# santi-pdp/segan_pytorch

Hardware: AMD Instinct MI355X
Metric: 16384-sample waveform chunks/sec (GAN step) (higher is better)
Workload: dtype f32

## Files before the change

include/segan_hip.h:

```cpp
#ifndef SEGAN_HIP_H
#define SEGAN_HIP_H

#include <stddef.h>
#include <stdint.h>

#ifdef __cplusplus
extern "C" {
#endif

#define SEGAN_ABI_VERSION 17

#define SEGAN_PAD_REFLECT 0
#define SEGAN_PAD_ZERO 1

#define SEGAN_ACT_NONE 0
#define SEGAN_ACT_TANH 1

typedef struct segan_src {
  const float* p0;
  const float* p1;
  int32_t C0;
  int32_t C1;
  const float* scale;
  const float* shift;
// ... 40 lines not shown

int segan_deconv1d_fwd(const segan_src* x, const void* wt, const float* w, const float* bias,
                       float* y, int B, int M, int N, int Ls, int K, int S, int pad, int act,
                       int precision, void* scratch, size_t scratch_bytes, void* stream);

int segan_deconv1d_dgrad(const float* dy, const void* wf, float* dx0, float* dx1, int B, int M,
                         int M0, int N, int Ls, int K, int S, int pad, int precision, void* scratch,
                         size_t scratch_bytes, void* stream);


int segan_bn_nsplit(int B, int C, int L);
int segan_bn_stats(const float* x, const float* gamma, const float* beta, float eps,
                   float momentum, float* running_mean, float* running_var, float* mean,
                   float* rstd, float* scale, float* shift, float* ws, int B, int C, int L,
                   void* stream);
int segan_bn_partial(const float* x, float* ws, int B, int C, int L, void* stream);
int segan_bn_final(const float* ws, int nsplit_total, const float* gamma, const float* beta,
                   float eps, float momentum, float* running_mean, float* running_var, float* mean,
                   float* rstd, float* scale, float* shift, int C, void* stream);

int segan_affine_tanh(const float* x, const float* scale, const float* shift, float* y, int B,
                      int C, int L, void* stream);
int segan_scale_mask(const float* x, const float* scale, const float* mask, float* y, int B, int C,
                     int L, void* stream);

int segan_affine_prelu(const float* x, const float* scale, const float* shift, const float* slope,
                       float* y, int B, int C, int L, void* stream);

int segan_sum_skip(const float* x0, const float* slope0, const float* x1, const float* alpha,
                   float* out, int B, int C, int L, void* stream);
// ... 169 lines not shown
```

segan_pytorch_amd/_lib.py:

```python
import ctypes
import os
from ctypes import POINTER, Structure, c_char_p, c_double, c_float, c_int, c_int32, c_int64, c_size_t, c_void_p

_HERE = os.path.dirname(os.path.abspath(__file__))
LIB_PATH = os.environ.get('SEGAN_HIP_LIB') or os.path.join(_HERE, 'libsegan_hip.so')

PAD_REFLECT = 0
PAD_ZERO = 1
ACT_NONE = 0
ACT_TANH = 1
ABI_VERSION = 17


class SeganSrc(Structure):
    _fields_ = [('p0', c_void_p), ('p1', c_void_p), ('C0', c_int32), ('C1', c_int32),
                ('scale', c_void_p), ('shift', c_void_p), ('slope', c_void_p)]


_P = c_void_p
_SRC = POINTER(SeganSrc)

SIGNATURES = {
    'segan_abi_version': (c_int, []),
    'segan_set_reserved_slots': (c_int, [c_int]),
# ... 9 lines not shown
    'segan_debug_last_wgrad': (None, [POINTER(c_int)]),
    'segan_conv1d_fwd': (c_int, [_SRC, _P, _P, _P, c_int, c_int, c_int, c_int, c_int, c_int, c_int,
                                 c_int, c_int, c_int, _P, c_size_t, _P]),
    'segan_conv1d_dgrad': (c_int, [_P, _P, _P, _P, _P, c_int, c_int, c_int, c_int, c_int, c_int, c_int,
                                   c_int, c_int, _P, c_size_t, _P]),
    'segan_wgrad': (c_int, [_SRC, _SRC, _P, c_int, c_int, c_int, c_int, c_int, c_int, c_int, c_int,
                            c_int, c_int, c_int, _P, c_size_t, _P]),
    'segan_wgrad_scratch_bytes': (c_size_t, [c_int, c_int, c_int, c_int, c_int, c_int, c_int]),
    'segan_deconv1d_fwd': (c_int, [_SRC, _P, _P, _P, _P, c_int, c_int, c_int, c_int, c_int, c_int, c_int,
                                   c_int, c_int, _P, c_size_t, _P]),
    'segan_deconv1d_dgrad': (c_int, [_P, _P, _P, _P, c_int, c_int, c_int, c_int, c_int, c_int, c_int,
                                     c_int, c_int, _P, c_size_t, _P]),
    'segan_bn_nsplit': (c_int, [c_int, c_int, c_int]),
    'segan_bn_stats': (c_int, [_P, _P, _P, c_float, c_float, _P, _P, _P, _P, _P, _P, _P, c_int, c_int,
                               c_int, _P]),
    'segan_bn_partial': (c_int, [_P, _P, c_int, c_int, c_int, _P]),
    'segan_bn_final': (c_int, [_P, c_int, _P, _P, c_float, c_float, _P, _P, _P, _P, _P, _P, c_int, _P]),
    'segan_act_bwd_bn_reduce': (c_int, [_P] * 12 + [c_int, c_int, c_int, _P]),
    'segan_act_bwd_bn_apply': (c_int, [_P] * 11 + [c_int, c_int, c_int, c_double, _P]),
    'segan_affine_prelu': (c_int, [_P, _P, _P, _P, _P, c_int, c_int, c_int, _P]),
    'segan_affine_tanh': (c_int, [_P, _P, _P, _P, c_int, c_int, c_int, _P]),
    'segan_scale_mask': (c_int, [_P, _P, _P, _P, c_int, c_int, c_int, _P]),
    'segan_sum_skip': (c_int, [_P, _P, _P, _P, _P, c_int, c_int, c_int, _P]),
    'segan_bce_logits_const': (c_int, [_P, c_float, _P, _P, _P, c_float, c_int, _P]),
    'segan_act_bwd': (c_int, [_P] * 16 + [c_int, c_int, c_int, _P]),
    'segan_tanh_bwd': (c_int, [_P, _P, _P, c_float, _P, _P, _P, c_int, c_int, c_int, _P]),
    'segan_gemm_scratch_bytes': (c_size_t, [c_int, c_int, c_int]),
    'segan_gemm': (c_int, [_P, c_int64, c_int64, _P, c_int64, c_int64, _P, c_int64, c_int, c_int,
                           c_int, c_int, c_int, _P, c_size_t, _P]),
    'segan_bias_prelu_rows': (c_int, [_P, _P, _P, _P, c_int, c_int, _P]),
# ... 105 lines not shown
```

segan_pytorch_amd/csrc/segan_pointwise.hip:

```cpp
#include "segan_common.h"

#define PW_THREADS 256

static int pw_nsplit(int B, int C, int L) {
  int ns = ceil_div(2048, C);
  if (ns > B) ns = B;
  long per = (long)B * L / ns;
  while (ns > 1 && per < 2048) {
    ns = (ns + 1) / 2;
    per = (long)B * L / ns;
  }
  return ns < 1 ? 1 : ns;
}

extern "C" int segan_bn_nsplit(int B, int C, int L) {
  if (B <= 0 || C <= 0 || L <= 0) return 0;
  return pw_nsplit(B, C, L);
}

template <int NV>
__device__ __forceinline__ void block_sum(float (&v)[NV], float* sm) {
  const int lane = threadIdx.x & 63, wave = threadIdx.x >> 6;
#pragma unroll
  for (int k = 0; k < NV; ++k) v[k] = warp_sum(v[k]);
// ... 23 lines not shown
  r.b_end = min(B, r.b_beg + per);
  return r;
}

__device__ __forceinline__ void chan_combine(float& n, float& mean, float& m2, float nb, float mb,
                                             float qb) {
  const float tot = n + nb;
  if (tot <= 0.0f) return;
  const float d = mb - mean;
  const float f = nb / tot;
  mean = fmaf(d, f, mean);
  m2 = m2 + qb + d * d * n * f;
  n = tot;
}

__global__ void bn_partial_kernel(const float* __restrict__ x, float* __restrict__ ws, int B, int C,
                                  int L, int nsplit) {
  __shared__ float sm[3 * (PW_THREADS / 64)];
  const ChanRange cr = chan_range(B, nsplit);
  const int nb = cr.b_end - cr.b_beg;
  const float* base = x + ((size_t)cr.b_beg * C + cr.c) * L;
  const size_t sstride = (size_t)C * L;
  const bool vec = (L & 3) == 0 && ((uintptr_t)x & 15) == 0;
  const int Lv = vec ? L >> 2 : L;
  int tr = PW_THREADS;
  while (tr > Lv && tr > 1) tr >>= 1;
  const int rp = PW_THREADS / tr;
  const int t0 = threadIdx.x % tr, r0 = threadIdx.x / tr;
  float K = 0.0f, s1 = 0.0f, s2 = 0.0f, n = 0.0f;
  if (r0 < nb && t0 < Lv) K = base[(size_t)r0 * sstride + (vec ? 4 * t0 : t0)];
  for (int b = r0; b < nb; b += rp) {
    const float* row = base + b * sstride;
// ... 24 lines not shown
    m2 = fmaxf(s2 - s1 * r, 0.0f);
  }
#pragma unroll
  for (int o = 32; o > 0; o >>= 1) {
    const float nb2 = __shfl_down(n, o, 64), mb2 = __shfl_down(mean, o, 64), qb2 = __shfl_down(m2, o, 64);
    chan_combine(n, mean, m2, nb2, mb2, qb2);
  }
  const int lane = threadIdx.x & 63, wave = threadIdx.x >> 6;
  if (lane == 0) {
    sm[3 * wave] = n; sm[3 * wave + 1] = mean; sm[3 * wave + 2] = m2;
  }
  __syncthreads();
  if (threadIdx.x == 0) {
    for (int w = 1; w < PW_THREADS / 64; ++w) chan_combine(n, mean, m2, sm[3 * w], sm[3 * w + 1], sm[3 * w + 2]);
    float* w = ws + ((size_t)blockIdx.y * C + cr.c) * 3;
    w[0] = n;
    w[1] = mean;
    w[2] = m2;
  }
}

__device__ __forceinline__ void bn_affine(float gamma, float beta, float mean, float rstd,
                                          float& scale, float& shift) {
  scale = gamma * rstd;
  shift = fmaf(-mean, scale, beta);
}

__global__ void bn_final_kernel(const float* __restrict__ ws, const float* gamma, const float* beta,
                                float eps, float momentum, float* running_mean, float* running_var,
                                float* mean_o, float* rstd_o, float* scale_o, float* shift_o, int C,
                                int nsplit) {
  const int c = blockIdx.x * blockDim.x + threadIdx.x;
  if (c >= C) return;
  double n = 0.0, mean = 0.0, m2 = 0.0;
  for (int s = 0; s < nsplit; ++s) {
    const float* w = ws + ((size_t)s * C + c) * 3;
    const double nb = w[0], mb = w[1], qb = w[2];
    if (nb <= 0.0) continue;
    const double tot = n + nb;
    const double d = mb - mean;
    mean += d * nb / tot;
    m2 += qb + d * d * n * nb / tot;
    n = tot;
  }
  const double var = n > 0 ? m2 / n : 0.0;
  const float rstd = (float)(1.0 / sqrt(var + (double)eps));
  const float g = gamma ? gamma[c] : 1.0f;
  const float bt = beta ? beta[c] : 0.0f;
  float sc, sh;
  bn_affine(g, bt, (float)mean, rstd, sc, sh);
  if (mean_o) mean_o[c] = (float)mean;
  if (rstd_o) rstd_o[c] = rstd;
  if (scale_o) scale_o[c] = sc;
  if (shift_o) shift_o[c] = sh;
  if (running_mean) running_mean[c] = (1.0f - momentum) * running_mean[c] + momentum * (float)mean;
  if (running_var) {
    const double unb = n > 1 ? m2 / (n - 1.0) : var;
    running_var[c] = (1.0f - momentum) * running_var[c] + momentum * (float)unb;
  }
}

extern "C" int segan_bn_stats(const float* x, const float* gamma, const float* beta, float eps,
                              float momentum, float* running_mean, float* running_var, float* mean,
                              float* rstd, float* scale, float* shift, float* ws, int B, int C,
                              int L, void* stream) {
  SEGAN_REQUIRE(x && ws, "bn_stats: NULL pointer");
  SEGAN_REQUIRE(B > 0 && C > 0 && L > 0, "bn_stats: bad sizes");
  hipStream_t st = (hipStream_t)stream;
  const int ns = pw_nsplit(B, C, L);
  hipLaunchKernelGGL(bn_partial_kernel, dim3(C, ns), dim3(PW_THREADS), 0, st, x, ws, B, C, L, ns);
  hipLaunchKernelGGL(bn_final_kernel, dim3(ceil_div(C, 64)), dim3(64), 0, st, ws, gamma, beta, eps,
                     momentum, running_mean, running_var, mean, rstd, scale, shift, C, ns);
  return segan_check_launch("bn_stats");
}

extern "C" int segan_bn_partial(const float* x, float* ws, int B, int C, int L, void* stream) {
  SEGAN_REQUIRE(x && ws, "bn_partial: NULL pointer");
  SEGAN_REQUIRE(B > 0 && C > 0 && L > 0, "bn_partial: bad sizes");
  const int ns = pw_nsplit(B, C, L);
  hipLaunchKernelGGL(bn_partial_kernel, dim3(C, ns), dim3(PW_THREADS), 0, (hipStream_t)stream, x, ws,
                     B, C, L, ns);
  return segan_check_launch("bn_partial");
}

extern "C" int segan_bn_final(const float* ws, int nsplit_total, const float* gamma,
                              const float* beta, float eps, float momentum, float* running_mean,
                              float* running_var, float* mean, float* rstd, float* scale,
                              float* shift, int C, void* stream) {
  SEGAN_REQUIRE(ws && nsplit_total > 0 && C > 0, "bn_final: bad arguments");
  hipLaunchKernelGGL(bn_final_kernel, dim3(ceil_div(C, 64)), dim3(64), 0, (hipStream_t)stream, ws,
                     gamma, beta, eps, momentum, running_mean, running_var, mean, rstd, scale, shift,
                     C, nsplit_total);
  return segan_check_launch("bn_final");
}

__global__ void affine_prelu_kernel(const float* __restrict__ x, const float* scale,
                                    const float* shift, const float* slope, float* __restrict__ y,
                                    size_t total, int C, int L) {
  for (size_t i = blockIdx.x * (size_t)blockDim.x + threadIdx.x; i < total;
       i += (size_t)gridDim.x * blockDim.x) {
    const int c = (int)((i / L) % C);
    float v = x[i];
    v = fmaf(v, scale ? scale[c] : 1.0f, shift ? shift[c] : 0.0f);
    if (slope) v = v > 0.f ? v : v * slope[c];
    y[i] = v;
  }
// ... 77 lines not shown

struct ActBwdArgs {
  const float* a;
  const float* dh;
  const float* dskip;
  const float* slope;
  const float* alpha;
  const float* mean;
  const float* rstd;
  const float* gamma;
  const float* beta;
  float* da;
  float* ws;
  int B, C, L, nsplit;
  float inv_count;
};

template <int PHASE>
__global__ void act_bwd_kernel(const ActBwdArgs p) {
  __shared__ float sm[16];
  const ChanRange cr = chan_range(p.B, p.nsplit);
  const int c = cr.c;
  const int nb = cr.b_end - cr.b_beg;
  const float sl = p.slope ? p.slope[c] : 1.0f;
  const float al = p.alpha ? p.alpha[c] : 0.0f;
  float mu = 0.f, rs = 1.f, ga = 1.f, be = 0.f, dbeta_m = 0.f, dgamma_m = 0.f, sc = 1.f, sh = 0.f;
  if (PHASE != 0) {
    mu = p.mean[c];
    rs = p.rstd[c];
    ga = p.gamma ? p.gamma[c] : 1.0f;
    be = p.beta ? p.beta[c] : 0.0f;
    bn_affine(ga, be, mu, rs, sc, sh);
  }
  if (PHASE == 2) {
    const float* tot = p.ws + (size_t)p.nsplit * p.C * 4 + (size_t)c * 2;
    dbeta_m = tot[0] * p.inv_count;
    dgamma_m = tot[1] * p.inv_count;
  }
  float r[3] = {0.f, 0.f, 0.f};
  const bool has_skip = p.dskip != nullptr;
  auto elem = [&](float av, float dh, float ds) -> float {
    if (PHASE == 0) {
      float g = dh * (av > 0.f ? 1.0f : sl);
      r[0] += dh * (av > 0.f ? 0.0f : av);
      if (has_skip) {
        g = fmaf(al, ds, g);
        r[1] = fmaf(ds, av, r[1]);
      }
      r[2] += g;
      return g;
    }
    const float xh = (av - mu) * rs;
// ... 29 lines not shown
        const f32x4 ds = has_skip ? *reinterpret_cast<const f32x4*>(p.dskip + i) : z4;
        f32x4 o;
#pragma unroll
        for (int e = 0; e < 4; ++e) o[e] = elem(av[e], dh[e], ds[e]);
        if (PHASE != 1) *reinterpret_cast<f32x4*>(p.da + i) = o;
      }
    } else {
      for (int t = t0; t < Lv; t += tr) {
        const size_t i = ro + t;
        const float o = elem(p.a[i], p.dh ? p.dh[i] : 0.0f, has_skip ? p.dskip[i] : 0.0f);
        if (PHASE != 1) p.da[i] = o;
      }
    }
  }
  block_sum<3>(r, sm);
  if (threadIdx.x == 0) {
    float* w = p.ws + ((size_t)blockIdx.y * p.C + c) * 4;
    w[0] = r[0];
    w[1] = r[1];
    w[2] = r[2];
  }
}

template <int PHASE>
__global__ void act_bwd_final_kernel(const ActBwdArgs p, float* dslope, float* dalpha,
                                     float* dgamma, float* dbeta, float* dbias) {
  const int c = blockIdx.x * blockDim.x + threadIdx.x;
  if (c >= p.C) return;
  float s0 = 0.f, s1 = 0.f, s2 = 0.f;
  for (int s = 0; s < p.nsplit; ++s) {
    const float* w = p.ws + ((size_t)s * p.C + c) * 4;
    s0 += w[0];
    s1 += w[1];
    s2 += w[2];
  }
// ... 13 lines not shown
  }
}

extern "C" int segan_act_bwd(const float* a, const float* dh, const float* dskip,
                             const float* slope, const float* alpha, const float* bn_mean,
                             const float* bn_rstd, const float* bn_gamma, const float* bn_beta,
                             float* da, float* dslope, float* dalpha, float* dgamma, float* dbeta,
                             float* dbias, float* ws, int B, int C, int L, void* stream) {
  SEGAN_REQUIRE(a && da && ws, "act_bwd: NULL pointer");
  SEGAN_REQUIRE(dh || dskip, "act_bwd: no incoming gradient");
  SEGAN_REQUIRE(B > 0 && C > 0 && L > 0, "act_bwd: bad sizes");
  SEGAN_REQUIRE((bn_mean == nullptr) == (bn_rstd == nullptr), "act_bwd: mean/rstd must pair");
  SEGAN_REQUIRE(!(dskip && !alpha), "act_bwd: dskip needs alpha");
  SEGAN_REQUIRE(!(bn_mean && dskip), "act_bwd: BN layers have no skip tap");
  hipStream_t st = (hipStream_t)stream;
  ActBwdArgs p;
  p.a = a; p.dh = dh; p.dskip = dskip; p.slope = slope; p.alpha = alpha;
  p.mean = bn_mean; p.rstd = bn_rstd; p.gamma = bn_gamma; p.beta = bn_beta;
  p.da = da; p.ws = ws; p.B = B; p.C = C; p.L = L;
  p.nsplit = pw_nsplit(B, C, L);
  p.inv_count = 1.0f / ((float)B * (float)L);
  const dim3 grid(C, p.nsplit), fgrid(ceil_div(C, 64));
  if (!bn_mean) {
    hipLaunchKernelGGL(act_bwd_kernel<0>, grid, dim3(PW_THREADS), 0, st, p);
    hipLaunchKernelGGL(act_bwd_final_kernel<0>, fgrid, dim3(64), 0, st, p, dslope, dalpha, dgamma,
                       dbeta, dbias);
  } else {
    hipLaunchKernelGGL(act_bwd_kernel<1>, grid, dim3(PW_THREADS), 0, st, p);
    hipLaunchKernelGGL(act_bwd_final_kernel<1>, fgrid, dim3(64), 0, st, p, dslope, dalpha, dgamma,
                       dbeta, dbias);
    hipLaunchKernelGGL(act_bwd_kernel<2>, grid, dim3(PW_THREADS), 0, st, p);
    hipLaunchKernelGGL(act_bwd_final_kernel<2>, fgrid, dim3(64), 0, st, p, dslope, dalpha, dgamma,
                       dbeta, dbias);
  }
  return segan_check_launch("act_bwd");
}

extern "C" int segan_act_bwd_bn_reduce(const float* a, const float* dh, const float* slope,
                                       const float* bn_mean, const float* bn_rstd,
                                       const float* bn_gamma, const float* bn_beta, float* dslope,
                                       float* dgamma, float* dbeta, float* totals, float* ws, int B,
                                       int C, int L, void* stream) {
  SEGAN_REQUIRE(a && dh && bn_mean && bn_rstd && totals && ws, "act_bwd_bn_reduce: NULL pointer");
  SEGAN_REQUIRE(B > 0 && C > 0 && L > 0, "act_bwd_bn_reduce: bad sizes");
  hipStream_t st = (hipStream_t)stream;
  ActBwdArgs p;
  p.a = a; p.dh = dh; p.dskip = nullptr; p.slope = slope; p.alpha = nullptr;
  p.mean = bn_mean; p.rstd = bn_rstd; p.gamma = bn_gamma; p.beta = bn_beta;
  p.da = nullptr; p.ws = ws; p.B = B; p.C = C; p.L = L;
  p.nsplit = pw_nsplit(B, C, L);
  p.inv_count = 1.0f / ((float)B * (float)L);
  hipLaunchKernelGGL(act_bwd_kernel<1>, dim3(C, p.nsplit), dim3(PW_THREADS), 0, st, p);
  hipLaunchKernelGGL(act_bwd_final_kernel<1>, dim3(ceil_div(C, 64)), dim3(64), 0, st, p, dslope,
                     (float*)nullptr, dgamma, dbeta, (float*)nullptr);
  if (hipMemcpyAsync(totals, ws + (size_t)p.nsplit * C * 4, (size_t)C * 2 * sizeof(float),
                     hipMemcpyDeviceToDevice, st) != hipSuccess) {
    segan_set_error("act_bwd_bn_reduce: copy of the totals failed");
    return SEGAN_ELAUNCH;
  }
  return segan_check_launch("act_bwd_bn_reduce");
}

extern "C" int segan_act_bwd_bn_apply(const float* a, const float* dh, const float* slope,
                                      const float* bn_mean, const float* bn_rstd,
                                      const float* bn_gamma, const float* bn_beta,
                                      const float* totals, float* da, float* dbias, float* ws, int B,
                                      int C, int L, double count_total, void* stream) {
  SEGAN_REQUIRE(a && dh && bn_mean && bn_rstd && totals && da && ws, "act_bwd_bn_apply: NULL pointer");
  SEGAN_REQUIRE(B > 0 && C > 0 && L > 0 && count_total >= (double)B * L, "act_bwd_bn_apply: bad sizes");
  hipStream_t st = (hipStream_t)stream;
  ActBwdArgs p;
  p.a = a; p.dh = dh; p.dskip = nullptr; p.slope = slope; p.alpha = nullptr;
  p.mean = bn_mean; p.rstd = bn_rstd; p.gamma = bn_gamma; p.beta = bn_beta;
  p.da = da; p.ws = ws; p.B = B; p.C = C; p.L = L;
  p.nsplit = pw_nsplit(B, C, L);
  p.inv_count = (float)(1.0 / count_total);
  if (hipMemcpyAsync(ws + (size_t)p.nsplit * C * 4, totals, (size_t)C * 2 * sizeof(float),
                     hipMemcpyDeviceToDevice, st) != hipSuccess) {
    segan_set_error("act_bwd_bn_apply: copy of the totals failed");
    return SEGAN_ELAUNCH;
  }
  hipLaunchKernelGGL(act_bwd_kernel<2>, dim3(C, p.nsplit), dim3(PW_THREADS), 0, st, p);
  hipLaunchKernelGGL(act_bwd_final_kernel<2>, dim3(ceil_div(C, 64)), dim3(64), 0, st, p,
                     (float*)nullptr, (float*)nullptr, (float*)nullptr, (float*)nullptr, dbias);
  return segan_check_launch("act_bwd_bn_apply");
}

__global__ void tanh_bwd_kernel(const float* __restrict__ y, const float* dy, const float* clean,
                                float l1_scale, float* __restrict__ da, float* ws, int B, int C,
                                int L, int nsplit) {
  __shared__ float sm[16];
  const ChanRange cr = chan_range(B, nsplit);
  const int nb = cr.b_end - cr.b_beg;
  const long cnt = (long)(nb > 0 ? nb : 0) * L;
  float r[1] = {0.f};
  for (long e = threadIdx.x; e < cnt; e += PW_THREADS) {
    const int b = cr.b_beg + (int)(e / L);
    const int t = (int)(e % L);
    const size_t i = ((size_t)b * C + cr.c) * L + t;
    const float yv = y[i];
    float g = dy ? dy[i] : 0.0f;
    if (clean) {
      const float d = yv - clean[i];
      g += l1_scale * (d > 0.f ? 1.0f : (d < 0.f ? -1.0f : 0.0f));
    }
    const float d = g * (1.0f - yv * yv);
    da[i] = d;
    r[0] += d;
  }
  block_sum<1>(r, sm);
  if (threadIdx.x == 0) ws[(size_t)blockIdx.y * C + cr.c] = r[0];
}

__global__ void sum_splits_add_kernel(const float* ws, float* out, int C, int nsplit) {
  const int c = blockIdx.x * blockDim.x + threadIdx.x;
  if (c >= C) return;
  float s = 0.f;
  for (int k = 0; k < nsplit; ++k) s += ws[(size_t)k * C + c];
  out[c] += s;
}

extern "C" int segan_tanh_bwd(const float* y, const float* dy, const float* clean, float l1_scale,
                              float* da, float* dbias, float* ws, int B, int C, int L,
                              void* stream) {
  SEGAN_REQUIRE(y && da && ws, "tanh_bwd: NULL pointer");
  SEGAN_REQUIRE(dy || clean, "tanh_bwd: no incoming gradient");
  SEGAN_REQUIRE(B > 0 && C > 0 && L > 0, "tanh_bwd: bad sizes");
  hipStream_t st = (hipStream_t)stream;
  const int ns = pw_nsplit(B, C, L);
  hipLaunchKernelGGL(tanh_bwd_kernel, dim3(C, ns), dim3(PW_THREADS), 0, st, y, dy, clean, l1_scale,
                     da, ws, B, C, L, ns);
  if (dbias)
    hipLaunchKernelGGL(sum_splits_add_kernel, dim3(ceil_div(C, 64)), dim3(64), 0, st, ws, dbias, C,
                       ns);
  return segan_check_launch("tanh_bwd");
}

__global__ void bias_prelu_rows_kernel(const float* __restrict__ x, const float* bias,
                                       const float* slope, float* __restrict__ y, int rows,
                                       int cols) {
  const size_t total = (size_t)rows * cols;
  for (size_t i = blockIdx.x * (size_t)blockDim.x + threadIdx.x; i < total;
       i += (size_t)gridDim.x * blockDim.x) {
    const int c = (int)(i % cols);
    float v = x[i] + (bias ? bias[c] : 0.0f);
    if (slope) v = v > 0.f ? v : v * slope[c];
    y[i] = v;
// ... 30 lines not shown
      s_b += d;
      dx[i] = d;
    }
  }
  sm[0][rg][cl] = s_sl;
  sm[1][rg][cl] = s_b;
  __syncthreads();
  if (rg == 0 && c < cols) {
    const float a = sm[0][0][cl] + sm[0][1][cl] + sm[0][2][cl] + sm[0][3][cl];
    const float b = sm[1][0][cl] + sm[1][1][cl] + sm[1][2][cl] + sm[1][3][cl];
    if (dslope && slope) dslope[c] += a;
    if (dbias) dbias[c] += b;
  }
}

extern "C" int segan_bias_prelu_rows_bwd(const float* x, const float* bias, const float* slope,
                                         const float* dy, float* dx, float* dslope, float* dbias,
                                         int rows, int cols, void* stream) {
  SEGAN_REQUIRE(x && dy && dx && rows > 0 && cols > 0, "bias_prelu_rows_bwd: bad arguments");
  hipLaunchKernelGGL(bias_prelu_rows_bwd_kernel, dim3(ceil_div(cols, 64)), dim3(256), 0,
                     (hipStream_t)stream, x, bias, slope, dy, dx, dslope, dbias, rows, cols);
  return segan_check_launch("bias_prelu_rows_bwd");
}

__global__ void mse_const_kernel(const float* __restrict__ x, float target, float* loss,
                                 float* grad, const float* gout, float gscale, int n) {
  __shared__ float sm[16];
  float r[1] = {0.f};
  const float inv = 1.0f / (float)n;
  if (gout) gscale *= gout[0];
  for (int i = threadIdx.x; i < n; i += PW_THREADS) {
    const float d = x[i] - target;
    r[0] = fmaf(d, d, r[0]);
    if (grad) grad[i] = 2.0f * d * inv * gscale;
  }
  block_sum<1>(r, sm);
// ... 288 lines not shown
```

segan_pytorch_amd/functional.py:

```python
import os

import torch

from . import ops
from .ops import ACT_NONE, ACT_TANH, PAD_REFLECT, PAD_ZERO, Src


def grad_buf(p):
    if p.grad is None:
        p.grad = torch.zeros_like(p, memory_format=torch.contiguous_format)
    elif not p.grad.is_contiguous():
        p.grad = p.grad.contiguous()
    return p.grad


def _gb(p, needed=True):
    if p is None or not needed or not p.requires_grad:
        return None
    return grad_buf(p)


def _bn_batch_stats(bn, training):
    return training or bn.running_mean is None or bn.running_var is None


def _bn_train_stats(c, bn, training=True):
    from . import distributed as sdist
    fn = sdist.bn_stats_sync if sdist.sync_bn_enabled() else ops.bn_stats
    track = training and bn.running_mean is not None and bn.running_var is not None
    momentum = 0.0
    if track:
        if bn.num_batches_tracked is not None:
            bn.num_batches_tracked += 1
        if bn.momentum is not None:
            momentum = bn.momentum
        else:
            momentum = 1.0 / float(bn.num_batches_tracked) if bn.num_batches_tracked is not None else 0.0
    return fn(c, bn.weight, bn.bias, bn.eps, momentum, bn.running_mean if track else None,
              bn.running_var if track else None)


def _bn_eval_affine(bn):
    rstd = torch.rsqrt(bn.running_var + bn.eps)
    gamma = bn.weight.detach() if bn.weight is not None else torch.ones_like(rstd)
    beta = bn.bias.detach() if bn.bias is not None else torch.zeros_like(rstd)
    scale = (gamma * rstd).contiguous()
# ... 816 lines not shown
```

segan_pytorch_amd/ops.py:

```python
import ctypes
import operator

import torch

from . import _lib
from . import layout
from ._lib import ACT_NONE, ACT_TANH, PAD_REFLECT, PAD_ZERO, SeganSrc, check


import os as _os

PREC_FP32, PREC_BF16, PREC_BF16X3 = 0, 1, 3
_PREC_NAMES = {'fp32': PREC_FP32, 'bf16': PREC_BF16, 'bf16x3': PREC_BF16X3}
_precision = _PREC_NAMES[_os.environ.get('SEGAN_PRECISION', 'fp32')]
_EUNSUPPORTED = -3


_deterministic = _os.environ.get('SEGAN_DETERMINISTIC', '0') == '1'


def set_deterministic(on):
    global _deterministic
    _deterministic = bool(on)

# ... 434 lines not shown
                                      _ptr(dx1), B, M, M0, N, Ls, K, S, pad, _precision, sp, sn,
                                      _stream())
        if rc != _EUNSUPPORTED:
            check(rc, 'deconv1d_dgrad')
            return dx0, dx1
    check(lib.segan_deconv1d_dgrad(_ptr(dy), _ptr(pack.f(w, S)), _ptr(dx0), _ptr(dx1), B, M, M0, N,
                                   Ls, K, S, pad, _fp32(), *_scratch(), _stream()), 'deconv1d_dgrad')
    return dx0, dx1


def _ws(B, C, L, per_split, extra, device):
    ns = _lib.load().segan_bn_nsplit(B, C, L)
    return torch.empty((per_split * ns * C + extra * C,), device=device, dtype=torch.float32)


def bn_stats(x, gamma, beta, eps, momentum, running_mean, running_var):
    _chk(x, 'x', 3)
    B, C, L = x.shape
    mean = torch.empty(C, device=x.device, dtype=torch.float32)
    rstd = torch.empty_like(mean)
    scale = torch.empty_like(mean)
    shift = torch.empty_like(mean)
    ws = _ws(B, C, L, 3, 0, x.device)
    check(_lib.load().segan_bn_stats(_ptr(x), _ptr(gamma), _ptr(beta), eps, momentum,
                                     _ptr(running_mean), _ptr(running_var), _ptr(mean), _ptr(rstd),
                                     _ptr(scale), _ptr(shift), _ptr(ws), B, C, L, _stream()),
          'bn_stats')
    return mean, rstd, scale, shift


def bn_partial(x):
    _chk(x, 'x', 3)
    B, C, L = x.shape
    ns = _lib.load().segan_bn_nsplit(B, C, L)
    ws = torch.empty((ns, C, 3), device=x.device, dtype=torch.float32)
    check(_lib.load().segan_bn_partial(_ptr(x), _ptr(ws), B, C, L, _stream()), 'bn_partial')
    return ws


def bn_final(ws_all, gamma, beta, eps, momentum, running_mean, running_var):
    _chk(ws_all, 'ws_all', 3)
    C = ws_all.shape[1]
    mean = torch.empty(C, device=ws_all.device, dtype=torch.float32)
# ... 980 lines not shown
```

Baseline: 3550.

## Fold split-reduction finalize kernels into producers via last-block ticket counters

```diff
diff --git a/include/segan_hip.h b/include/segan_hip.h
--- a/include/segan_hip.h
+++ b/include/segan_hip.h
@@ -78,6 +78,10 @@
                    float momentum, float* running_mean, float* running_var, float* mean,
                    float* rstd, float* scale, float* shift, float* ws, int B, int C, int L,
                    void* stream);
+int segan_bn_stats_tracked(const float* x, const float* gamma, const float* beta, float eps,
+                           float momentum, float* running_mean, float* running_var,
+                           int64_t* num_batches_tracked, float* mean, float* rstd, float* scale,
+                           float* shift, float* ws, int B, int C, int L, void* stream);
 int segan_bn_partial(const float* x, float* ws, int B, int C, int L, void* stream);
 int segan_bn_final(const float* ws, int nsplit_total, const float* gamma, const float* beta,
                    float eps, float momentum, float* running_mean, float* running_var, float* mean,
diff --git a/segan_pytorch_amd/_lib.py b/segan_pytorch_amd/_lib.py
--- a/segan_pytorch_amd/_lib.py
+++ b/segan_pytorch_amd/_lib.py
@@ -47,6 +47,8 @@
     'segan_bn_nsplit': (c_int, [c_int, c_int, c_int]),
     'segan_bn_stats': (c_int, [_P, _P, _P, c_float, c_float, _P, _P, _P, _P, _P, _P, _P, c_int, c_int,
                                c_int, _P]),
+    'segan_bn_stats_tracked': (c_int, [_P, _P, _P, c_float, c_float, _P, _P, _P, _P, _P, _P, _P, _P, c_int,
+                                       c_int, c_int, _P]),
     'segan_bn_partial': (c_int, [_P, _P, c_int, c_int, c_int, _P]),
     'segan_bn_final': (c_int, [_P, c_int, _P, _P, c_float, c_float, _P, _P, _P, _P, _P, _P, c_int, _P]),
     'segan_act_bwd_bn_reduce': (c_int, [_P] * 12 + [c_int, c_int, c_int, _P]),
diff --git a/segan_pytorch_amd/csrc/segan_pointwise.hip b/segan_pytorch_amd/csrc/segan_pointwise.hip
--- a/segan_pytorch_amd/csrc/segan_pointwise.hip
+++ b/segan_pytorch_amd/csrc/segan_pointwise.hip
@@ -1,6 +1,94 @@
 #include "segan_common.h"
+#include <mutex>
+#include <stdlib.h>
 
 #define PW_THREADS 256
+
+#define PW_TICKET_WORDS 16384
+#define PW_TICKET_STREAMS 64
+
+static bool pw_fold_on() {
+  const char* e = getenv("SEGAN_LAUNCH_FOLD");
+  return !(e && e[0] == '0');
+}
+
+struct PwTicketBlock {
+  int dev;
+  hipStream_t st;
+  unsigned* p;
+};
+static PwTicketBlock pw_ticket_blocks[PW_TICKET_STREAMS];
+static int pw_ticket_nblocks = 0;
+static std::mutex pw_ticket_mu;
+
+static unsigned* pw_tickets(hipStream_t st, int words) {
+  if (!pw_fold_on() || words > PW_TICKET_WORDS) return nullptr;
+  int dev = 0;
+  if (hipGetDevice(&dev) != hipSuccess) return nullptr;
+  std::lock_guard<std::mutex> lock(pw_ticket_mu);
+  for (int i = 0; i < pw_ticket_nblocks; ++i)
+    if (pw_ticket_blocks[i].dev == dev && pw_ticket_blocks[i].st == st) return pw_ticket_blocks[i].p;
+  if (pw_ticket_nblocks == PW_TICKET_STREAMS) return nullptr;
+  hipStreamCaptureStatus cs = hipStreamCaptureStatusNone;
+  if (hipStreamIsCapturing(st, &cs) != hipSuccess || cs != hipStreamCaptureStatusNone) {
+    (void)hipGetLastError();
+    return nullptr;
+  }
+  unsigned* p = nullptr;
+  if (hipMalloc(&p, PW_TICKET_WORDS * sizeof(unsigned)) != hipSuccess ||
+      hipMemset(p, 0, PW_TICKET_WORDS * sizeof(unsigned)) != hipSuccess ||
+      hipDeviceSynchronize() != hipSuccess) {
+    (void)hipGetLastError();
+    if (p) (void)hipFree(p);
+    return nullptr;
+  }
+  pw_ticket_blocks[pw_ticket_nblocks++] = {dev, st, p};
+  return p;
+}
+
+__device__ __forceinline__ void pw_publish(float* p, float v) {
+  __hip_atomic_store(p, v, __ATOMIC_RELAXED, __HIP_MEMORY_SCOPE_AGENT);
+}
+__device__ __forceinline__ float pw_collect(const float* p) {
+  return __hip_atomic_load(const_cast<float*>(p), __ATOMIC_RELAXED, __HIP_MEMORY_SCOPE_AGENT);
+}
+__device__ __forceinline__ bool pw_arrive_last(unsigned* ticket, int n) {
+  asm volatile("s_waitcnt vmcnt(0)" ::: "memory");
+  const unsigned t = __hip_atomic_fetch_add(ticket, 1u, __ATOMIC_RELAXED, __HIP_MEMORY_SCOPE_AGENT);
+  if (t != (unsigned)(n - 1)) return false;
+  __builtin_amdgcn_fence(__ATOMIC_ACQUIRE, "agent");
+  asm volatile("s_waitcnt vmcnt(0)" ::: "memory");
+  return true;
+}
+__device__ __forceinline__ void pw_ticket_reset(unsigned* ticket) {
+  __hip_atomic_store(ticket, 0u, __ATOMIC_RELAXED, __HIP_MEMORY_SCOPE_AGENT);
+}
+__device__ __forceinline__ bool pw_wave_arrive_last(unsigned* ticket, int n) {
+  int last = 0;
+  if ((threadIdx.x & 63) == 0) last = pw_arrive_last(ticket, n) ? 1 : 0;
+  return __builtin_amdgcn_readfirstlane(last) != 0;
+}
+__device__ __forceinline__ float pw_lane(float v, int lane) {
+  return __int_as_float(__builtin_amdgcn_readlane(__float_as_int(v), lane));
+}
+template <int NV, bool COLLECT>
+__device__ __forceinline__ void pw_sum_splits(const float* base, size_t stride, int nsplit,
+                                              float (&s)[NV]) {
+  const int lane = threadIdx.x & 63;
+#pragma unroll
+  for (int k = 0; k < NV; ++k) s[k] = 0.f;
+  for (int s0 = 0; s0 < nsplit; s0 += 64) {
+    float v[NV];
+    const float* w = base + (size_t)(s0 + lane) * stride;
+#pragma unroll
+    for (int k = 0; k < NV; ++k)
+      v[k] = s0 + lane < nsplit ? (COLLECT ? pw_collect(w + k) : w[k]) : 0.f;
+    const int cnt = min(64, nsplit - s0);
+    for (int j = 0; j < cnt; ++j)
+#pragma unroll
+      for (int k = 0; k < NV; ++k) s[k] += pw_lane(v[k], j);
+  }
+}
 
 static int pw_nsplit(int B, int C, int L) {
   int ns = ceil_div(2048, C);
@@ -61,8 +149,82 @@
   n = tot;
 }
 
-__global__ void bn_partial_kernel(const float* __restrict__ x, float* __restrict__ ws, int B, int C,
-                                  int L, int nsplit) {
+__device__ __forceinline__ void bn_affine(float gamma, float beta, float mean, float rstd,
+                                          float& scale, float& shift) {
+  scale = gamma * rstd;
+  shift = fmaf(-mean, scale, beta);
+}
+
+struct BnFinalArgs {
+  const float* gamma;
+  const float* beta;
+  float eps, momentum;
+  float* running_mean;
+  float* running_var;
+  float* mean_o;
+  float* rstd_o;
+  float* scale_o;
+  float* shift_o;
+  long long* tracked;
+};
+
+template <bool FOLDED>
+__device__ __forceinline__ void bn_finalize(const float* ws, const BnFinalArgs& f, int c, int C,
+                                            int nsplit) {
+  double n = 0.0, mean = 0.0, m2 = 0.0;
+  auto merge = [&](double nb, double mb, double qb) {
+    if (nb <= 0.0) return;
+    const double tot = n + nb;
+    const double d = mb - mean;
+    mean += d * nb / tot;
+    m2 += qb + d * d * n * nb / tot;
+    n = tot;
+  };
+  if (FOLDED) {
+    const int lane = threadIdx.x & 63;
+    for (int s0 = 0; s0 < nsplit; s0 += 64) {
+      const float* w = ws + ((size_t)(s0 + lane) * C + c) * 3;
+      const bool in = s0 + lane < nsplit;
+      const float v0 = in ? pw_collect(w) : 0.f, v1 = in ? pw_collect(w + 1) : 0.f,
+                  v2 = in ? pw_collect(w + 2) : 0.f;
+      const int cnt = min(64, nsplit - s0);
+      for (int j = 0; j < cnt; ++j) merge(pw_lane(v0, j), pw_lane(v1, j), pw_lane(v2, j));
+    }
+    if (lane != 0) return;
+  } else {
+    for (int s = 0; s < nsplit; ++s) {
+      const float* w = ws + ((size_t)s * C + c) * 3;
+      merge(w[0], w[1], w[2]);
+    }
+  }
+  const double var = n > 0 ? m2 / n : 0.0;
+  const float rstd = (float)(1.0 / sqrt(var + (double)f.eps));
+  const float g = f.gamma ? f.gamma[c] : 1.0f;
+  const float bt = f.beta ? f.beta[c] : 0.0f;
+  float sc, sh;
+  bn_affine(g, bt, (float)mean, rstd, sc, sh);
+  if (f.mean_o) f.mean_o[c] = (float)mean;
+  if (f.rstd_o) f.rstd_o[c] = rstd;
+  if (f.scale_o) f.scale_o[c] = sc;
+  if (f.shift_o) f.shift_o[c] = sh;
+  if (f.running_mean)
+    f.running_mean[c] = (1.0f - f.momentum) * f.running_mean[c] + f.momentum * (float)mean;
+  if (f.running_var) {
+    const double unb = n > 1 ? m2 / (n - 1.0) : var;
+    f.running_var[c] = (1.0f - f.momentum) * f.running_var[c] + f.momentum * (float)unb;
+  }
+  if (f.tracked && c == 0) f.tracked[0] += 1;
+}
+
+__global__ void bn_final_kernel(const float* __restrict__ ws, const BnFinalArgs f, int C,
+                                int nsplit) {
+  const int c = blockIdx.x * blockDim.x + threadIdx.x;
+  if (c >= C) return;
+  bn_finalize<false>(ws, f, c, C, nsplit);
+}
+
+__global__ void bn_partial_kernel(const float* __restrict__ x, float* ws, int B, int C, int L,
+                                  int nsplit, unsigned* tickets, const BnFinalArgs f) {
   __shared__ float sm[3 * (PW_THREADS / 64)];
   const ChanRange cr = chan_range(B, nsplit);
   const int nb = cr.b_end - cr.b_beg;
@@ -117,50 +279,31 @@
   if (threadIdx.x == 0) {
     for (int w = 1; w < PW_THREADS / 64; ++w) chan_combine(n, mean, m2, sm[3 * w], sm[3 * w + 1], sm[3 * w + 2]);
     float* w = ws + ((size_t)blockIdx.y * C + cr.c) * 3;
-    w[0] = n;
-    w[1] = mean;
-    w[2] = m2;
-  }
-}
-
-__device__ __forceinline__ void bn_affine(float gamma, float beta, float mean, float rstd,
-                                          float& scale, float& shift) {
-  scale = gamma * rstd;
-  shift = fmaf(-mean, scale, beta);
-}
-
-__global__ void bn_final_kernel(const float* __restrict__ ws, const float* gamma, const float* beta,
-                                float eps, float momentum, float* running_mean, float* running_var,
-                                float* mean_o, float* rstd_o, float* scale_o, float* shift_o, int C,
-                                int nsplit) {
-  const int c = blockIdx.x * blockDim.x + threadIdx.x;
-  if (c >= C) return;
-  double n = 0.0, mean = 0.0, m2 = 0.0;
-  for (int s = 0; s < nsplit; ++s) {
-    const float* w = ws + ((size_t)s * C + c) * 3;
-    const double nb = w[0], mb = w[1], qb = w[2];
-    if (nb <= 0.0) continue;
-    const double tot = n + nb;
-    const double d = mb - mean;
-    mean += d * nb / tot;
-    m2 += qb + d * d * n * nb / tot;
-    n = tot;
-  }
-  const double var = n > 0 ? m2 / n : 0.0;
-  const float rstd = (float)(1.0 / sqrt(var + (double)eps));
-  const float g = gamma ? gamma[c] : 1.0f;
-  const float bt = beta ? beta[c] : 0.0f;
-  float sc, sh;
-  bn_affine(g, bt, (float)mean, rstd, sc, sh);
-  if (mean_o) mean_o[c] = (float)mean;
-  if (rstd_o) rstd_o[c] = rstd;
-  if (scale_o) scale_o[c] = sc;
-  if (shift_o) shift_o[c] = sh;
-  if (running_mean) running_mean[c] = (1.0f - momentum) * running_mean[c] + momentum * (float)mean;
-  if (running_var) {
-    const double unb = n > 1 ? m2 / (n - 1.0) : var;
-    running_var[c] = (1.0f - momentum) * running_var[c] + momentum * (float)unb;
-  }
+    if (!tickets) {
+      w[0] = n;
+      w[1] = mean;
+      w[2] = m2;
+    } else {
+      pw_publish(w, n);
+      pw_publish(w + 1, mean);
+      pw_publish(w + 2, m2);
+    }
+  }
+  if (tickets && threadIdx.x < 64 && pw_wave_arrive_last(tickets + cr.c, nsplit)) {
+    bn_finalize<true>(ws, f, cr.c, C, nsplit);
+    if (threadIdx.x == 0) pw_ticket_reset(tickets + cr.c);
+  }
+}
+
+static int bn_stats_launch(const float* x, float* ws, int B, int C, int L, const BnFinalArgs& f,
+                           hipStream_t st, const char* what) {
+  const int ns = pw_nsplit(B, C, L);
+  unsigned* tickets = pw_tickets(st, C);
+  hipLaunchKernelGGL(bn_partial_kernel, dim3(C, ns), dim3(PW_THREADS), 0, st, x, ws, B, C, L, ns,
+                     tickets, f);
+  if (!tickets)
+    hipLaunchKernelGGL(bn_final_kernel, dim3(ceil_div(C, 64)), dim3(64), 0, st, ws, f, C, ns);
+  return segan_check_launch(what);
 }
 
 extern "C" int segan_bn_stats(const float* x, const float* gamma, const float* beta, float eps,
@@ -169,12 +312,21 @@
                               int L, void* stream) {
   SEGAN_REQUIRE(x && ws, "bn_stats: NULL pointer");
   SEGAN_REQUIRE(B > 0 && C > 0 && L > 0, "bn_stats: bad sizes");
-  hipStream_t st = (hipStream_t)stream;
-  const int ns = pw_nsplit(B, C, L);
-  hipLaunchKernelGGL(bn_partial_kernel, dim3(C, ns), dim3(PW_THREADS), 0, st, x, ws, B, C, L, ns);
-  hipLaunchKernelGGL(bn_final_kernel, dim3(ceil_div(C, 64)), dim3(64), 0, st, ws, gamma, beta, eps,
-                     momentum, running_mean, running_var, mean, rstd, scale, shift, C, ns);
-  return segan_check_launch("bn_stats");
+  const BnFinalArgs f = {gamma, beta, eps, momentum, running_mean, running_var,
+                         mean, rstd, scale, shift, nullptr};
+  return bn_stats_launch(x, ws, B, C, L, f, (hipStream_t)stream, "bn_stats");
+}
+
+extern "C" int segan_bn_stats_tracked(const float* x, const float* gamma, const float* beta,
+                                      float eps, float momentum, float* running_mean,
+                                      float* running_var, int64_t* num_batches_tracked, float* mean,
+                                      float* rstd, float* scale, float* shift, float* ws, int B,
+                                      int C, int L, void* stream) {
+  SEGAN_REQUIRE(x && ws, "bn_stats_tracked: NULL pointer");
+  SEGAN_REQUIRE(B > 0 && C > 0 && L > 0, "bn_stats_tracked: bad sizes");
+  const BnFinalArgs f = {gamma, beta, eps, momentum, running_mean, running_var,
+                         mean, rstd, scale, shift, (long long*)num_batches_tracked};
+  return bn_stats_launch(x, ws, B, C, L, f, (hipStream_t)stream, "bn_stats_tracked");
 }
 
 extern "C" int segan_bn_partial(const float* x, float* ws, int B, int C, int L, void* stream) {
@@ -182,7 +334,7 @@
   SEGAN_REQUIRE(B > 0 && C > 0 && L > 0, "bn_partial: bad sizes");
   const int ns = pw_nsplit(B, C, L);
   hipLaunchKernelGGL(bn_partial_kernel, dim3(C, ns), dim3(PW_THREADS), 0, (hipStream_t)stream, x, ws,
-                     B, C, L, ns);
+                     B, C, L, ns, (unsigned*)nullptr, BnFinalArgs{});
   return segan_check_launch("bn_partial");
 }
 
@@ -191,8 +343,9 @@
                               float* running_var, float* mean, float* rstd, float* scale,
                               float* shift, int C, void* stream) {
   SEGAN_REQUIRE(ws && nsplit_total > 0 && C > 0, "bn_final: bad arguments");
-  hipLaunchKernelGGL(bn_final_kernel, dim3(ceil_div(C, 64)), dim3(64), 0, (hipStream_t)stream, ws,
-                     gamma, beta, eps, momentum, running_mean, running_var, mean, rstd, scale, shift,
+  const BnFinalArgs f = {gamma, beta, eps, momentum, running_mean, running_var,
+                         mean, rstd, scale, shift, nullptr};
+  hipLaunchKernelGGL(bn_final_kernel, dim3(ceil_div(C, 64)), dim3(64), 0, (hipStream_t)stream, ws, f,
                      C, nsplit_total);
   return segan_check_launch("bn_final");
 }
@@ -300,6 +453,12 @@
   float* ws;
   int B, C, L, nsplit;
   float inv_count;
+  unsigned* tickets;
+  float* dslope;
+  float* dalpha;
+  float* dgamma;
+  float* dbeta;
+  float* dbias;
 };
 
 template <int PHASE>
@@ -319,9 +478,21 @@
     bn_affine(ga, be, mu, rs, sc, sh);
   }
   if (PHASE == 2) {
-    const float* tot = p.ws + (size_t)p.nsplit * p.C * 4 + (size_t)c * 2;
-    dbeta_m = tot[0] * p.inv_count;
-    dgamma_m = tot[1] * p.inv_count;
+    if (p.tickets) {
+      float t[3];
+      pw_sum_splits<3, false>(p.ws + (size_t)c * 4, (size_t)p.C * 4, p.nsplit, t);
+      if (blockIdx.y == 0 && threadIdx.x == 0) {
+        if (p.dslope) p.dslope[c] += t[0];
+        if (p.dbeta) p.dbeta[c] += t[1];
+        if (p.dgamma) p.dgamma[c] += t[2];
+      }
+      dbeta_m = t[1] * p.inv_count;
+      dgamma_m = t[2] * p.inv_count;
+    } else {
+      const float* tot = p.ws + (size_t)p.nsplit * p.C * 4 + (size_t)c * 2;
+      dbeta_m = tot[0] * p.inv_count;
+      dgamma_m = tot[1] * p.inv_count;
+    }
   }
   float r[3] = {0.f, 0.f, 0.f};
   const bool has_skip = p.dskip != nullptr;
@@ -381,11 +552,36 @@
     }
   }
   block_sum<3>(r, sm);
+  const bool fold = p.tickets && PHASE != 1;
   if (threadIdx.x == 0) {
     float* w = p.ws + ((size_t)blockIdx.y * p.C + c) * 4;
-    w[0] = r[0];
-    w[1] = r[1];
-    w[2] = r[2];
+    if (!fold) {
+      w[0] = r[0];
+      w[1] = r[1];
+      w[2] = r[2];
+    } else if (PHASE == 0) {
+      pw_publish(w, r[0]);
+      pw_publish(w + 1, r[1]);
+      pw_publish(w + 2, r[2]);
+    } else {
+      pw_publish(w + 3, r[0]);
+    }
+  }
+  if (fold && threadIdx.x < 64 && pw_wave_arrive_last(p.tickets + c, p.nsplit)) {
+    if (PHASE == 0) {
+      float t[3];
+      pw_sum_splits<3, true>(p.ws + (size_t)c * 4, (size_t)p.C * 4, p.nsplit, t);
+      if (threadIdx.x == 0) {
+        if (p.dslope) p.dslope[c] += t[0];
+        if (p.dalpha) p.dalpha[c] += t[1];
+        if (p.dbias) p.dbias[c] += t[2];
+      }
+    } else {
+      float t[1];
+      pw_sum_splits<1, true>(p.ws + (size_t)c * 4 + 3, (size_t)p.C * 4, p.nsplit, t);
+      if (threadIdx.x == 0 && p.dbias) p.dbias[c] += t[0];
+    }
+    if (threadIdx.x == 0) pw_ticket_reset(p.tickets + c);
   }
 }
 
@@ -429,14 +625,23 @@
   SEGAN_REQUIRE(!(dskip && !alpha), "act_bwd: dskip needs alpha");
   SEGAN_REQUIRE(!(bn_mean && dskip), "act_bwd: BN layers have no skip tap");
   hipStream_t st = (hipStream_t)stream;
-  ActBwdArgs p;
+  ActBwdArgs p = {};
   p.a = a; p.dh = dh; p.dskip = dskip; p.slope = slope; p.alpha = alpha;
   p.mean = bn_mean; p.rstd = bn_rstd; p.gamma = bn_gamma; p.beta = bn_beta;
   p.da = da; p.ws = ws; p.B = B; p.C = C; p.L = L;
   p.nsplit = pw_nsplit(B, C, L);
   p.inv_count = 1.0f / ((float)B * (float)L);
+  p.tickets = pw_tickets(st, C);
+  p.dslope = dslope; p.dalpha = dalpha; p.dgamma = dgamma; p.dbeta = dbeta; p.dbias = dbias;
   const dim3 grid(C, p.nsplit), fgrid(ceil_div(C, 64));
-  if (!bn_mean) {
+  if (p.tickets) {
+    if (!bn_mean) {
+      hipLaunchKernelGGL(act_bwd_kernel<0>, grid, dim3(PW_THREADS), 0, st, p);
+    } else {
+      hipLaunchKernelGGL(act_bwd_kernel<1>, grid, dim3(PW_THREADS), 0, st, p);
+      hipLaunchKernelGGL(act_bwd_kernel<2>, grid, dim3(PW_THREADS), 0, st, p);
+    }
+  } else if (!bn_mean) {
     hipLaunchKernelGGL(act_bwd_kernel<0>, grid, dim3(PW_THREADS), 0, st, p);
     hipLaunchKernelGGL(act_bwd_final_kernel<0>, fgrid, dim3(64), 0, st, p, dslope, dalpha, dgamma,
                        dbeta, dbias);
@@ -459,10 +664,11 @@
   SEGAN_REQUIRE(a && dh && bn_mean && bn_rstd && totals && ws, "act_bwd_bn_reduce: NULL pointer");
   SEGAN_REQUIRE(B > 0 && C > 0 && L > 0, "act_bwd_bn_reduce: bad sizes");
   hipStream_t st = (hipStream_t)stream;
-  ActBwdArgs p;
+  ActBwdArgs p = {};
   p.a = a; p.dh = dh; p.dskip = nullptr; p.slope = slope; p.alpha = nullptr;
   p.mean = bn_mean; p.rstd = bn_rstd; p.gamma = bn_gamma; p.beta = bn_beta;
   p.da = nullptr; p.ws = ws; p.B = B; p.C = C; p.L = L;
+  p.tickets = nullptr;
   p.nsplit = pw_nsplit(B, C, L);
   p.inv_count = 1.0f / ((float)B * (float)L);
   hipLaunchKernelGGL(act_bwd_kernel<1>, dim3(C, p.nsplit), dim3(PW_THREADS), 0, st, p);
@@ -484,10 +690,11 @@
   SEGAN_REQUIRE(a && dh && bn_mean && bn_rstd && totals && da && ws, "act_bwd_bn_apply: NULL pointer");
   SEGAN_REQUIRE(B > 0 && C > 0 && L > 0 && count_total >= (double)B * L, "act_bwd_bn_apply: bad sizes");
   hipStream_t st = (hipStream_t)stream;
-  ActBwdArgs p;
+  ActBwdArgs p = {};
   p.a = a; p.dh = dh; p.dskip = nullptr; p.slope = slope; p.alpha = nullptr;
   p.mean = bn_mean; p.rstd = bn_rstd; p.gamma = bn_gamma; p.beta = bn_beta;
   p.da = da; p.ws = ws; p.B = B; p.C = C; p.L = L;
+  p.tickets = nullptr;
   p.nsplit = pw_nsplit(B, C, L);
   p.inv_count = (float)(1.0 / count_total);
   if (hipMemcpyAsync(ws + (size_t)p.nsplit * C * 4, totals, (size_t)C * 2 * sizeof(float),
@@ -503,7 +710,7 @@
 
 __global__ void tanh_bwd_kernel(const float* __restrict__ y, const float* dy, const float* clean,
                                 float l1_scale, float* __restrict__ da, float* ws, int B, int C,
-                                int L, int nsplit) {
+                                int L, int nsplit, unsigned* tickets, float* dbias) {
   __shared__ float sm[16];
   const ChanRange cr = chan_range(B, nsplit);
   const int nb = cr.b_end - cr.b_beg;
@@ -524,7 +731,19 @@
     r[0] += d;
   }
   block_sum<1>(r, sm);
-  if (threadIdx.x == 0) ws[(size_t)blockIdx.y * C + cr.c] = r[0];
+  if (threadIdx.x == 0) {
+    float* w = ws + (size_t)blockIdx.y * C + cr.c;
+    if (!tickets) w[0] = r[0];
+    else pw_publish(w, r[0]);
+  }
+  if (tickets && threadIdx.x < 64 && pw_wave_arrive_last(tickets + cr.c, nsplit)) {
+    float t[1];
+    pw_sum_splits<1, true>(ws + cr.c, (size_t)C, nsplit, t);
+    if (threadIdx.x == 0) {
+      dbias[cr.c] += t[0];
+      pw_ticket_reset(tickets + cr.c);
+    }
+  }
 }
 
 __global__ void sum_splits_add_kernel(const float* ws, float* out, int C, int nsplit) {
@@ -543,9 +762,10 @@
   SEGAN_REQUIRE(B > 0 && C > 0 && L > 0, "tanh_bwd: bad sizes");
   hipStream_t st = (hipStream_t)stream;
   const int ns = pw_nsplit(B, C, L);
+  unsigned* tickets = dbias ? pw_tickets(st, C) : nullptr;
   hipLaunchKernelGGL(tanh_bwd_kernel, dim3(C, ns), dim3(PW_THREADS), 0, st, y, dy, clean, l1_scale,
-                     da, ws, B, C, L, ns);
-  if (dbias)
+                     da, ws, B, C, L, ns, tickets, dbias);
+  if (dbias && !tickets)
     hipLaunchKernelGGL(sum_splits_add_kernel, dim3(ceil_div(C, 64)), dim3(64), 0, st, ws, dbias, C,
                        ns);
   return segan_check_launch("tanh_bwd");
@@ -606,12 +826,61 @@
   }
 }
 
+#define ROWS_IN_FLIGHT 16
+__global__ __launch_bounds__(256) void bias_prelu_rows_bwd_batched_kernel(
+    const float* __restrict__ x, const float* bias, const float* slope,
+    const float* __restrict__ dy, float* __restrict__ dx, float* dslope, float* dbias, int rows,
+    int cols) {
+  __shared__ float sm[2][4][64];
+  const int cl = threadIdx.x & 63, rg = threadIdx.x >> 6;
+  const int c = blockIdx.x * 64 + cl;
+  float s_sl = 0.f, s_b = 0.f;
+  if (c < cols) {
+    const float bs = bias ? bias[c] : 0.0f;
+    const float sl = slope ? slope[c] : 1.0f;
+    for (int r0 = rg; r0 < rows; r0 += 4 * ROWS_IN_FLIGHT) {
+      float xv[ROWS_IN_FLIGHT], gv[ROWS_IN_FLIGHT];
+#pragma unroll
+      for (int u = 0; u < ROWS_IN_FLIGHT; ++u) {
+        const size_t i = (size_t)min(r0 + 4 * u, rows - 1) * cols + c;
+        xv[u] = x[i];
+        gv[u] = dy[i];
+      }
+#pragma unroll
+      for (int u = 0; u < ROWS_IN_FLIGHT; ++u) {
+        const int r = r0 + 4 * u;
+        if (r < rows) {
+          const float v = xv[u] + bs;
+          const float g = gv[u];
+          const float d = g * (v > 0.f ? 1.0f : sl);
+          s_sl += g * (v > 0.f ? 0.0f : v);
+          s_b += d;
+          dx[(size_t)r * cols + c] = d;
+        }
+      }
+    }
+  }
+  sm[0][rg][cl] = s_sl;
+  sm[1][rg][cl] = s_b;
+  __syncthreads();
+  if (rg == 0 && c < cols) {
+    const float a = sm[0][0][cl] + sm[0][1][cl] + sm[0][2][cl] + sm[0][3][cl];
+    const float b = sm[1][0][cl] + sm[1][1][cl] + sm[1][2][cl] + sm[1][3][cl];
+    if (dslope && slope) dslope[c] += a;
+    if (dbias) dbias[c] += b;
+  }
+}
+
 extern "C" int segan_bias_prelu_rows_bwd(const float* x, const float* bias, const float* slope,
                                          const float* dy, float* dx, float* dslope, float* dbias,
                                          int rows, int cols, void* stream) {
   SEGAN_REQUIRE(x && dy && dx && rows > 0 && cols > 0, "bias_prelu_rows_bwd: bad arguments");
-  hipLaunchKernelGGL(bias_prelu_rows_bwd_kernel, dim3(ceil_div(cols, 64)), dim3(256), 0,
-                     (hipStream_t)stream, x, bias, slope, dy, dx, dslope, dbias, rows, cols);
+  if (pw_fold_on())
+    hipLaunchKernelGGL(bias_prelu_rows_bwd_batched_kernel, dim3(ceil_div(cols, 64)), dim3(256), 0,
+                       (hipStream_t)stream, x, bias, slope, dy, dx, dslope, dbias, rows, cols);
+  else
+    hipLaunchKernelGGL(bias_prelu_rows_bwd_kernel, dim3(ceil_div(cols, 64)), dim3(256), 0,
+                       (hipStream_t)stream, x, bias, slope, dy, dx, dslope, dbias, rows, cols);
   return segan_check_launch("bias_prelu_rows_bwd");
 }
 
diff --git a/segan_pytorch_amd/functional.py b/segan_pytorch_amd/functional.py
--- a/segan_pytorch_amd/functional.py
+++ b/segan_pytorch_amd/functional.py
@@ -30,6 +30,10 @@
     track = training and bn.running_mean is not None and bn.running_var is not None
     momentum = 0.0
     if track:
+        if (bn.momentum is not None and bn.num_batches_tracked is not None and c.is_cuda
+                and fn is ops.bn_stats and ops.launch_fold()):
+            return ops.bn_stats_tracked(c, bn.weight, bn.bias, bn.eps, bn.momentum, bn.running_mean,
+                                        bn.running_var, bn.num_batches_tracked)
         if bn.num_batches_tracked is not None:
             bn.num_batches_tracked += 1
         if bn.momentum is not None:
diff --git a/segan_pytorch_amd/ops.py b/segan_pytorch_amd/ops.py
--- a/segan_pytorch_amd/ops.py
+++ b/segan_pytorch_amd/ops.py
@@ -472,7 +472,11 @@
     return torch.empty((per_split * ns * C + extra * C,), device=device, dtype=torch.float32)
 
 
-def bn_stats(x, gamma, beta, eps, momentum, running_mean, running_var):
+def launch_fold():
+    return _os.environ.get('SEGAN_LAUNCH_FOLD', '1')[:1] != '0'
+
+
+def _bn_stats(x, gamma, beta, eps, momentum, running_mean, running_var, tracked):
     _chk(x, 'x', 3)
     B, C, L = x.shape
     mean = torch.empty(C, device=x.device, dtype=torch.float32)
@@ -480,11 +484,27 @@
     scale = torch.empty_like(mean)
     shift = torch.empty_like(mean)
     ws = _ws(B, C, L, 3, 0, x.device)
-    check(_lib.load().segan_bn_stats(_ptr(x), _ptr(gamma), _ptr(beta), eps, momentum,
-                                     _ptr(running_mean), _ptr(running_var), _ptr(mean), _ptr(rstd),
-                                     _ptr(scale), _ptr(shift), _ptr(ws), B, C, L, _stream()),
-          'bn_stats')
+    if tracked is not None:
+        if tracked.dtype != torch.int64 or tracked.device != x.device:
+            raise ValueError('bn_stats_tracked: num_batches_tracked must be an int64 tensor on x.device')
+        check(_lib.load().segan_bn_stats_tracked(
+            _ptr(x), _ptr(gamma), _ptr(beta), eps, momentum, _ptr(running_mean), _ptr(running_var),
+            _ptr(tracked), _ptr(mean), _ptr(rstd), _ptr(scale), _ptr(shift), _ptr(ws), B, C, L,
+            _stream()), 'bn_stats_tracked')
+    else:
+        check(_lib.load().segan_bn_stats(_ptr(x), _ptr(gamma), _ptr(beta), eps, momentum,
+                                         _ptr(running_mean), _ptr(running_var), _ptr(mean), _ptr(rstd),
+                                         _ptr(scale), _ptr(shift), _ptr(ws), B, C, L, _stream()),
+              'bn_stats')
     return mean, rstd, scale, shift
+
+
+def bn_stats(x, gamma, beta, eps, momentum, running_mean, running_var):
+    return _bn_stats(x, gamma, beta, eps, momentum, running_mean, running_var, None)
+
+
+def bn_stats_tracked(x, gamma, beta, eps, momentum, running_mean, running_var, num_batches_tracked):
+    return _bn_stats(x, gamma, beta, eps, momentum, running_mean, running_var, num_batches_tracked)
 
 
 def bn_partial(x):
```

Result: no change. 3560 (median of 6 runs) (+0.3%).
